# JanLohse/raw2film

Measured on AMD Instinct MI355X. Metric: megapixels/sec full film pipeline (neg+print+grain+halation+MTF), 100MP frame, higher is better.
Workload: dtype f32 (pointwise stages, grain) + f64 (FFT stencils; the MTF's scratch images are complex64)

## Files before the change

### raw2film_amd/csrc/r2f_fft.hip

```cpp
#include <algorithm>

#include "r2f_launch.h"
#include "r2f_fft_math.h"

#include "../../include/r2f.h"

namespace r2f {

constexpr int kN = kFftN;
constexpr int kFftThreads = 256;
constexpr int kTPitch = 17;
constexpr int kTLine = 16 * kTPitch;

#ifndef R2F_FFT_EXPT
#define R2F_FFT_EXPT 0
#endif
template <bool INV>
__device__ __forceinline__ void fft256(cplx (&v)[16], const cplx w1, double* tbuf, int lane) {
    dft16<INV>(v);
    twiddle_powers<INV>(v, w1);
    if (R2F_FFT_EXPT & 1) {
        dft16<INV>(v);
        return;
    }
// ... 119 lines not shown
    __builtin_amdgcn_wave_barrier();
#pragma unroll
    for (int i = 0; i < 16; ++i) v[i] = make_double2(re[i], rd[4 * i]);
    __builtin_amdgcn_wave_barrier();
    dft16<INV>(v);
    const cplx wh = make_double2(h == 0 ? 1.0 : (h == 1 ? 0.9951847266721969 : (h == 2 ? 0.9807852804032304 : 0.9569403357322088)),
                                 h == 0 ? 0.0 : (h == 1 ? -0.0980171403295606 : (h == 2 ? -0.19509032201612825 : -0.2902846772544623)));
    twiddle_powers<INV>(v, wh);
    const bool upper = h & 2, odd = h & 1, rot = h == 3;
#pragma unroll
    for (int c = 0; c < 16; ++c) {
        cplx o = make_double2(swap_lane2(v[c].x), swap_lane2(v[c].y));
        cplx b = upper ? csub(o, v[c]) : cadd(v[c], o);
        if (rot) b = INV ? make_double2(-b.y, b.x) : make_double2(b.y, -b.x);
        o = make_double2(swap_lane1(b.x), swap_lane1(b.y));
        v[c] = odd ? csub(o, b) : cadd(b, o);
    }
}

__device__ __forceinline__ bool window_of(const FftConvArgs& a, int t, int& wy, int& wx) {
    if (t >= a.ntiles) return false;
    const int ty = a.y0 + (t / a.gx) * a.vy, tx = (t % a.gx) * a.vx;
    wy = ty - a.ay;
    wx = tx - a.ax;
    return true;
}

__device__ __forceinline__ double* wave_tbuf(double* smem) { return smem + (threadIdx.x >> 6) * 4 * kTLine; }

__device__ __forceinline__ unsigned sidx(int r, int k, int nbx) {
    return (unsigned)((((r >> 4) * nbx + (k >> 4)) << 8) + ((((k >> 2) & 3) * 16 + (r & 15)) << 2) + (k & 3));
}

__device__ __forceinline__ cplx& at(cplx* base, unsigned idx) {
    return *reinterpret_cast<cplx*>(reinterpret_cast<char*>(base) + (idx << 4));
}
__device__ __forceinline__ const cplx& at(const cplx* base, unsigned idx) {
    return *reinterpret_cast<const cplx*>(reinterpret_cast<const char*>(base) + (idx << 4));
}

struct __attribute__((packed, aligned(4))) C96 {
    unsigned hr, hi;
    unsigned lo;
};
template <int ST>
__device__ __forceinline__ cplx sld(const void* base, unsigned idx) {
    if (ST == 1) {
        const float2 v = *reinterpret_cast<const float2*>(reinterpret_cast<const char*>(base) + (idx << 3));
        return make_double2((double)v.x, (double)v.y);
    }
    if (ST == 2) {
        const C96 e = *reinterpret_cast<const C96*>(reinterpret_cast<const char*>(base) + idx * 12u);
        return make_double2(__hiloint2double((int)e.hr, (int)(e.lo << 16)), __hiloint2double((int)e.hi, (int)(e.lo & 0xffff0000u)));
    }
    return *reinterpret_cast<const cplx*>(reinterpret_cast<const char*>(base) + (idx << 4));
}
template <int ST>
__device__ __forceinline__ void sst(void* base, unsigned idx, const cplx v) {
    if (ST == 1)
        *reinterpret_cast<float2*>(reinterpret_cast<char*>(base) + (idx << 3)) = make_float2((float)v.x, (float)v.y);
    else if (ST == 2) {
        const unsigned long long br = (unsigned long long)__double_as_longlong(v.x) + 0x8000ull;
        const unsigned long long bi = (unsigned long long)__double_as_longlong(v.y) + 0x8000ull;
        C96 e;
        e.hr = (unsigned)(br >> 32), e.hi = (unsigned)(bi >> 32);
        e.lo = ((unsigned)br >> 16) | ((unsigned)bi & 0xffff0000u);
        *reinterpret_cast<C96*>(reinterpret_cast<char*>(base) + idx * 12u) = e;
    } else
        *reinterpret_cast<cplx*>(reinterpret_cast<char*>(base) + (idx << 4)) = v;
}
__device__ __forceinline__ bool pair_packed(const FftConvArgs& a, int pc) { return a.dyn_flags[pc] != 0; }

template <int ST>
__device__ __forceinline__ char* simg(double2* s1, long long pair, long long n) {
    return reinterpret_cast<char*>(s1) + pair * n * (ST == 1 ? 8 : (ST == 2 ? 12 : 16));
}

#ifndef R2F_DECIDE_OWN_COLUMNS_ONLY
#define R2F_DECIDE_OWN_COLUMNS_ONLY 0
#endif
__device__ __forceinline__ void reflected_reach(int w0, int n, int size, int& lo, int& hi) {
    const int last = size - 1, w1 = w0 + n - 1;
    lo = max(w0, 0), hi = min(w1, last);
    if (w0 < 0) hi = max(hi, min(-w0, last));
    if (w1 > last) lo = min(lo, max(2 * last - w1, 0));
}
__global__ __launch_bounds__(256) void fft_decide_kernel(const FftConvArgs a, const RangeRecord rec, const float bound, const float floor_, int* flags) {
    const int pc = blockIdx.x * 256 + threadIdx.x;
    if (pc >= a.ppc) return;
    int lo = (int)kFrameMinReset, hi = 0;
    bool known = rec.tiles != nullptr && !(rec.blk && rec.blk->e_max == 0x7f800000u);
    for (int half = 0; half < 2 && known; ++half) {
        int wy, wx;
        if (!window_of(a, 2 * pc + half, wy, wx)) continue;
        const int b0 = a.src.gy0, b1 = a.src.gy0 + a.src.rows - 1;
        const int r0 = clampi(max(wy, 0), b0, b1), r1 = clampi(min(wy + a.ny - 1, a.H_global - 1), b0, b1);
        int c0, c1;
        reflected_reach(wx, a.nx, a.W, c0, c1);
#if R2F_DECIDE_OWN_COLUMNS_ONLY
        c0 = max(wx, 0), c1 = min(wx + a.nx - 1, a.W - 1);
#endif
        for (int ty = r0 >> kRangeTileRowsLog2; ty <= (r1 >> kRangeTileRowsLog2); ++ty)
// ... 4 lines not shown
                }
                const int2 t = rec.tiles[(long long)ty * rec.txn + tx];
                if (t.x == (int)kFrameMinReset && t.y == (int)kFrameMaxReset) known = false;
                lo = min(lo, t.x), hi = max(hi, t.y);
            }
    }
    const float flo = __int_as_float(lo), fhi = __int_as_float(hi);
    flags[pc] = (known && fhi <= bound * fmaxf(flo, floor_)) ? 1 : 0;
}

#ifndef R2F_FFT_EXP
#define R2F_FFT_EXP 0
#endif
template <int XL>
struct RowGeom {
    static constexpr int NX = 256 << XL, NBX = NX / 16, LPL = 16 << XL, ROWS = kFftThreads / LPL;
    static __device__ __forceinline__ int out_col(int l, int q) {
        return XL == 2 ? (l >> 2) + 16 * q + 256 * (((l & 1) << 1) | ((l >> 1) & 1)) : (XL == 1 ? 256 * (l & 1) + 16 * q + (l >> 1) : l + 16 * q);
    }
    static __device__ __forceinline__ double* line_buf(double* wave_buf, int lane) {
        return XL == 2 ? wave_buf : wave_buf + (XL == 1 ? (lane >> 5) * kTLine512 : (lane >> 4) * kTLine);
    }
    template <bool INV>
    static __device__ __forceinline__ void fft(cplx (&v)[16], const FftConvArgs& a, int l, double* wave_buf, int lane) {
        if (XL == 2)
            fft1024<INV>(v, a.tw1024[l], wave_buf, lane);
        else if (XL == 1)
            fft512<INV>(v, a.tw512[l], wave_buf, lane);
        else
            fft256<INV>(v, a.tw[l], wave_buf, lane);
    }
};

template <int XL, int ST>
__device__ __forceinline__ void fft_rows_fwd_body(const FftConvArgs& a, double* fsm) {
    typedef RowGeom<XL> G;
    constexpr int NX = G::NX, LPL = G::LPL;
    const int lane = threadIdx.x & 63, l = lane & (LPL - 1);
    unsigned tid0 = threadIdx.x;
    asm volatile("" : "+v"(tid0));
    const int pair = blockIdx.y, r = blockIdx.x * G::ROWS + tid0 / LPL;
    int wyA = 0, wxA = 0, wyB = 0, wxB = 0;
    const int gp = a.pair0 + pair, ci = gp / a.ppc, pc = gp - ci * a.ppc;
    const bool hasA = window_of(a, 2 * pc, wyA, wxA), hasB = window_of(a, 2 * pc + 1, wyB, wxB);
    const float* src = a.src.data + (long long)a.chan[ci] * a.src.plane_stride;
    if (R2F_FFT_EXP & 8) {
        const int above = pair - (a.gx + 1) / 2;
        if ((int)(blockIdx.x + 1) * G::ROWS <= a.ny - a.vy && above >= 0 && (a.pair0 + above) / a.ppc == ci && !a.raw) return;
    }
    cplx v[16];
    if (R2F_FFT_EXP & 1) {
#pragma unroll
        for (int m = 0; m < 16; ++m) v[m] = make_double2(1.0 + m + l, 0.5 * r);
    } else if (a.raw) {
#pragma unroll
        for (int m = 0; m < 16; ++m) v[m] = make_double2((double)src[(long long)r * NX + l + LPL * m], 0.0);
    } else {
        const float* rowA = src;
        const float* rowB = src;
        if (hasA) {
            const int sy = reflect101(wyA + r, a.H_global) - a.src.gy0;
            rowA = src + (long long)clampi(sy, 0, a.src.rows - 1) * a.W;
        }
        if (hasB) {
            const int sy = reflect101(wyB + r, a.H_global) - a.src.gy0;
            rowB = src + (long long)clampi(sy, 0, a.src.rows - 1) * a.W;
        }
        const bool inA = wxA >= 0 && wxA + NX <= a.W, inB = wxB >= 0 && wxB + NX <= a.W;
        float fa[16], fb[16];
#pragma unroll
        for (int m = 0; m < 16; ++m) fa[m] = fb[m] = 0.f;
        if (hasA) {
            if (inA) {
                const float* pa = rowA + wxA + l;
#pragma unroll
                for (int m = 0; m < 16; ++m) fa[m] = pa[LPL * m];
            } else {
#pragma unroll
                for (int m = 0; m < 16; ++m) fa[m] = rowA[reflect101(wxA + l + LPL * m, a.W)];
            }
        }
        if (hasB) {
            if (inB) {
                const float* pb = rowB + wxB + l;
#pragma unroll
                for (int m = 0; m < 16; ++m) fb[m] = pb[LPL * m];
            } else {
#pragma unroll
                for (int m = 0; m < 16; ++m) fb[m] = rowB[reflect101(wxB + l + LPL * m, a.W)];
            }
        }
#pragma unroll
        for (int m = 0; m < 16; ++m) v[m] = make_double2(__builtin_isfinite(fa[m]) ? (double)fa[m] : 0.0, __builtin_isfinite(fb[m]) ? (double)fb[m] : 0.0);
    }
    bool packed = false;
    if (ST == 3) packed = pair_packed(a, pc);
    if (!(R2F_FFT_EXP & 4)) {
        G::template fft<false>(v, a, l, wave_tbuf(fsm), lane);
    }
    unsigned tid = threadIdx.x;
    asm volatile("" : "+v"(tid));
    const int rs = blockIdx.x * G::ROWS + tid / LPL;
    const unsigned sb = sidx(rs, G::out_col(l, 0), G::NBX);
    if (ST == 3) {
        char* s1 = simg<3>(a.s1, pair, (long long)a.ny * NX);
        if (packed) {
#pragma unroll
            for (int q = 0; q < 16; ++q) sst<2>(s1, sb + q * 256, v[q]);
        } else {
#pragma unroll
            for (int q = 0; q < 16; ++q) sst<0>(s1, sb + q * 256, v[q]);
        }
        return;
    }
    constexpr int STS = ST == 3 ? 0 : ST;
    char* s1 = simg<STS>(a.s1, pair, (long long)a.ny * NX);
    if (R2F_FFT_EXP & 2) {
        if (v[3].x == 1.2345e300) sst<STS>(s1, 0, v[5]);
        return;
    }
#pragma unroll
    for (int q = 0; q < 16; ++q) sst<STS>(s1, sb + q * 256, v[q]);
    if (R2F_FFT_EXP & 8) {
        const int below = pair + (a.gx + 1) / 2;
        if (r >= a.vy && below < a.npairs && (a.pair0 + below) / a.ppc == ci && !a.raw) {
            char* s2 = simg<STS>(a.s1, below, (long long)a.ny * NX);
#pragma unroll
            for (int q = 0; q < 16; ++q) sst<STS>(s2, sidx(r - a.vy, G::out_col(l, q), G::NBX), v[q]);
        }
    }
}

#ifndef R2F_FFT_WPE1
#define R2F_FFT_WPE1 4
#endif
template <int XL, int ST>
__global__ __launch_bounds__(kFftThreads) __attribute__((amdgpu_waves_per_eu(R2F_FFT_WPE1, 8))) void fft_rows_fwd_kernel(const FftConvArgs a) {
    extern __shared__ __attribute__((aligned(16))) double fsm[];
    fft_rows_fwd_body<XL, ST>(a, fsm);
}

#ifndef R2F_FFT_EXP2
#define R2F_FFT_EXP2 0
#endif
__device__ __forceinline__ double& rat(cplx* base, unsigned idx) {
    return *reinterpret_cast<double*>(reinterpret_cast<char*>(base) + (idx << 3));
}
__device__ __forceinline__ double rat(const cplx* base, unsigned idx) {
    return *reinterpret_cast<const double*>(reinterpret_cast<const char*>(base) + (idx << 3));
}

template <int NBX, int ST, bool KR>
__device__ __forceinline__ void fft_cols_body(const FftConvArgs& a, const int mode, double* fsm) {
    const int lane = threadIdx.x & 63, l = lane & 15;
    const int pair = blockIdx.y, k = blockIdx.x * 16 + (threadIdx.x >> 4);
    char* s1 = simg<ST>(a.s1, pair, (long long)kN * (NBX * 16));
    const cplx* kf = a.kfs[(a.pair0 + pair) / a.ppc];
#ifndef R2F_FFT_KR_EARLY
#define R2F_FFT_KR_EARLY 0
#endif
    constexpr bool kEarly = (R2F_FFT_KR_EARLY >> (ST == 1 ? 1 : 0)) & 1;
    double kr[16];
    if (KR && kEarly && mode != 1) {
#pragma unroll
        for (int q = 0; q < 16; ++q) kr[q] = (R2F_FFT_EXP2 & 4) ? 0.5 + 0.25 * q : rat(kf, sidx(l + 16 * q, k, NBX));
    }
    cplx v[16];
#pragma unroll
    for (int m = 0; m < 16; ++m) v[m] = (R2F_FFT_EXP2 & 1) ? make_double2(1.0 + m + l, 0.5 * k) : sld<ST>(s1, sidx(l + 16 * m, k, NBX));
    const cplx w1 = a.tw[l];
    double* tbuf = wave_tbuf(fsm);
    fft256<false>(v, w1, tbuf, lane);
    if (mode == 1) {
        const double sc = R2F_FFT_EPI2 ? 1.0 / ((double)kN * (NBX * 16)) : 1.0;
#pragma unroll
        for (int q = 0; q < 16; ++q) {
            if (KR)
                rat(a.kf_out, sidx(l + 16 * q, k, NBX)) = v[q].x * sc;
            else
                at(a.kf_out, sidx(l + 16 * q, k, NBX)) = make_double2(v[q].x * sc, -v[q].y * sc);
        }
        return;
    }
    if (KR) {
        if (!kEarly) {
#pragma unroll
            for (int q = 0; q < 16; ++q) kr[q] = (R2F_FFT_EXP2 & 4) ? 0.5 + 0.25 * q : rat(kf, sidx(l + 16 * q, k, NBX));
        }
#pragma unroll
        for (int q = 0; q < 16; ++q) v[q] = make_double2(v[q].x * kr[q], v[q].y * kr[q]);
    } else {
#pragma unroll
        for (int q = 0; q < 16; ++q) v[q] = cmul(v[q], (R2F_FFT_EXP2 & 4) ? make_double2(0.5, 0.25 * q) : at(kf, sidx(l + 16 * q, k, NBX)));
    }
    fft256<true>(v, w1, tbuf, lane);
    if (R2F_FFT_EXP2 & 2) {
        if (v[3].x == 1.2345e300) sst<ST>(s1, 0, v[5]);
        return;
    }
#pragma unroll
    for (int q = 0; q < 16; ++q)
        if ((unsigned)(l + 16 * q - a.oy) < (unsigned)a.vy) sst<ST>(s1, sidx(l + 16 * q, k, NBX), v[q]);
}

template <int NBX, int ST, bool KR>
__device__ __forceinline__ void fft_cols_y512_body(const FftConvArgs& a, const int mode, double* fsm) {
    const int lane = threadIdx.x & 63, l = lane & 31;
    const int pair = blockIdx.y, k = blockIdx.x * 8 + (threadIdx.x >> 5);
    char* s1 = simg<ST>(a.s1, pair, (long long)512 * (NBX * 16));
    cplx v[16];
#pragma unroll
    for (int m = 0; m < 16; ++m) v[m] = sld<ST>(s1, sidx(l + 32 * m, k, NBX));
    const cplx w1 = a.tw512[l];
    double* tbuf = wave_tbuf(fsm);
    fft512<false>(v, w1, tbuf, lane);
    const cplx* kf = a.kfs[(a.pair0 + pair) / a.ppc];
    const int f0 = 256 * (l & 1) + (l >> 1);
    if (mode == 1) {
        const double sc = R2F_FFT_EPI2 ? 1.0 / (512.0 * (NBX * 16)) : 1.0;
#pragma unroll
        for (int q = 0; q < 16; ++q) {
            if (KR)
                rat(a.kf_out, sidx(f0 + 16 * q, k, NBX)) = v[q].x * sc;
            else
                at(a.kf_out, sidx(f0 + 16 * q, k, NBX)) = make_double2(v[q].x * sc, -v[q].y * sc);
        }
        return;
    }
    if (KR) {
        double kr[16];
#pragma unroll
        for (int q = 0; q < 16; ++q) kr[q] = rat(kf, sidx(f0 + 16 * q, k, NBX));
#pragma unroll
        for (int q = 0; q < 16; ++q) v[q] = make_double2(v[q].x * kr[q], v[q].y * kr[q]);
    } else {
#pragma unroll
        for (int q = 0; q < 16; ++q) v[q] = cmul(v[q], at(kf, sidx(f0 + 16 * q, k, NBX)));
    }
    fft512_rev<true>(v, w1, tbuf, lane);
#pragma unroll
    for (int q = 0; q < 16; ++q)
        if ((unsigned)(l + 32 * q - a.oy) < (unsigned)a.vy) sst<ST>(s1, sidx(l + 32 * q, k, NBX), v[q]);
}

#ifndef R2F_FFT_WPE2
#define R2F_FFT_WPE2 2
#endif
template <int NBX, bool Y512, int ST, bool KR>
__global__ __launch_bounds__(kFftThreads) __attribute__((amdgpu_waves_per_eu(R2F_FFT_WPE2, 8))) void fft_cols_kernel(const FftConvArgs a, const int mode) {
    extern __shared__ __attribute__((aligned(16))) double fsm[];
    if (Y512)
        fft_cols_y512_body<NBX, ST, KR>(a, mode, fsm);
    else
        fft_cols_body<NBX, ST, KR>(a, mode, fsm);
}


template <int NBX, int ST>
__device__ __forceinline__ void fft_cols_walk_body(const FftConvArgs& a, double* fsm) {
    const int lane = threadIdx.x & 63, l = lane & 15;
    const int k = blockIdx.x * 16 + (threadIdx.x >> 4);
    double* tbuf = wave_tbuf(fsm);
    const long long img = (long long)kN * (NBX * 16);
    const int G = gridDim.y;
    const cplx w1 = a.tw[l];
    double kr[16];
    int ci_have = -1;
    for (int pair = blockIdx.y; pair < a.npairs; pair += G) {
        const int gp = a.pair0 + pair, ci = gp / a.ppc;
        const bool packed = ST == 3 ? pair_packed(a, gp - ci * a.ppc) : false;
        char* s1 = simg<ST>(a.s1, pair, img);
        unsigned sbase = sidx(l, k, NBX);
        cplx w = w1;
        asm volatile("" : "+v"(w.x), "+v"(w.y), "+v"(sbase));
        if (ci != ci_have) {
// ... 16 lines not shown
#pragma unroll
            for (int m = 0; m < 16; ++m) v[m] = sld<STL>(s1, sbase + m * (NBX * 256));
        }
        fft256<false>(v, w, tbuf, lane);
#pragma unroll
        for (int q = 0; q < 16; ++q) v[q] = make_double2(v[q].x * kr[q], v[q].y * kr[q]);
        asm volatile("" : "+v"(w.x), "+v"(w.y));
        fft256<true>(v, w, tbuf, lane);
        if (ST == 3) {
            if (packed) {
#pragma unroll
                for (int q = 0; q < 16; ++q)
                    if ((unsigned)(l + 16 * q - a.oy) < (unsigned)a.vy) sst<2>(s1, sbase + q * (NBX * 256), v[q]);
            } else {
#pragma unroll
                for (int q = 0; q < 16; ++q)
                    if ((unsigned)(l + 16 * q - a.oy) < (unsigned)a.vy) sst<0>(s1, sbase + q * (NBX * 256), v[q]);
            }
        } else {
            constexpr int STS = ST == 3 ? 0 : ST;
#pragma unroll
            for (int q = 0; q < 16; ++q)
                if ((unsigned)(l + 16 * q - a.oy) < (unsigned)a.vy) sst<STS>(s1, sbase + q * (NBX * 256), v[q]);
        }
    }
}

template <int NBX, int ST>
__global__ __launch_bounds__(kFftThreads) __attribute__((amdgpu_waves_per_eu(2, 2))) void fft_cols_walk_kernel(const FftConvArgs a) {
    extern __shared__ __attribute__((aligned(16))) double fsm[];
    fft_cols_walk_body<NBX, ST>(a, fsm);
}

#ifndef R2F_FFT_EXP3
#define R2F_FFT_EXP3 0
#endif
#ifndef R2F_FFT_CURVE_BATCH
#define R2F_FFT_CURVE_BATCH 4
#endif
template <int XL, int EPI, int ST>
__device__ __forceinline__ void fft_rows_inv_body(const FftConvArgs& a, double* fsm) {
    typedef RowGeom<XL> G;
    constexpr int NX = G::NX, LPL = G::LPL;
    const int lane = threadIdx.x & 63, l = lane & (LPL - 1);
    const int pair = blockIdx.y, r = (a.oy & ~(G::ROWS - 1)) + blockIdx.x * G::ROWS + threadIdx.x / LPL, ro = r - a.oy;
    const bool live = (unsigned)ro < (unsigned)a.vy;
    bool packed = false;
    if (ST == 3) packed = pair_packed(a, (a.pair0 + pair) % a.ppc);
    float4* cells_lds = reinterpret_cast<float4*>(fsm + a.epi_lds_off);
    if (EPI == 2) {
        const int gp0 = a.pair0 + pair, ch0 = a.chan[gp0 / a.ppc];
        const float4* src_cells = a.curve.cells + (long long)ch0 * (a.curve.m - 1);
        for (int i = threadIdx.x; i < a.curve.m - 1; i += kFftThreads) cells_lds[i] = src_cells[i];
        __syncthreads();
    }
    cplx v[16];
    if (R2F_FFT_EXP3 & 1) {
#pragma unroll
        for (int m = 0; m < 16; ++m) v[m] = make_double2(1.0 + m + l, 0.5 * r);
    } else if (ST == 3) {
        const char* s1 = simg<3>(a.s1, pair, (long long)a.ny * NX);
        if (packed) {
#pragma unroll
            for (int m = 0; m < 16; ++m) v[m] = sld<2>(s1, sidx(live ? r : a.oy, l + LPL * m, G::NBX));
        } else {
#pragma unroll
            for (int m = 0; m < 16; ++m) v[m] = sld<0>(s1, sidx(live ? r : a.oy, l + LPL * m, G::NBX));
        }
    } else {
        constexpr int STL = ST == 3 ? 0 : ST;
        const char* s1 = simg<STL>(a.s1, pair, (long long)a.ny * NX);
#pragma unroll
        for (int m = 0; m < 16; ++m) v[m] = sld<STL>(s1, sidx(live ? r : a.oy, l + LPL * m, G::NBX));
    }
    if (!(R2F_FFT_EXP3 & 4)) {
        G::template fft<true>(v, a, l, wave_tbuf(fsm), lane);
    }
    if (!live) return;
    if (R2F_FFT_EXP3 & 2) {
        if (v[3].x == 1.2345e300) a.dst.data[0] = (float)v[5].y;
        return;
    }
    const int gp = a.pair0 + pair, ci = gp / a.ppc, pc = gp - ci * a.ppc, ch = a.chan[ci];
    float* dplane = a.dst.data + (long long)ch * a.dst.plane_stride;
    const double scale = R2F_FFT_EPI2 ? 1.0 : 1.0 / ((double)NX * a.ny);
#pragma unroll
    for (int half = 0; half < 2; ++half) {
        int wy, wx;
        if (!window_of(a, 2 * pc + half, wy, wx)) continue;
        const int gy = wy + a.ay + ro;
        if (gy >= a.y1) continue;
        float* dbase = dplane + (long long)(gy - a.dst.gy0) * a.W + wx + a.ax;
        float o[16];
#pragma unroll
        for (int q = 0; q < 16; ++q) o[q] = R2F_FFT_EPI2 ? (float)(half ? v[q].y : v[q].x) : (float)((half ? v[q].y : v[q].x) * scale);
        if (EPI) {
            constexpr int CB = R2F_FFT_CURVE_BATCH;
#pragma unroll
            for (int b = 0; b < 16 / CB; ++b) {
                float ob[CB];
#ifndef R2F_FFT_EPI_ABLATE
#define R2F_FFT_EPI_ABLATE 0
#endif
#pragma unroll
                for (int q = 0; q < CB; ++q) ob[q] = (R2F_FFT_EPI_ABLATE & 6) ? o[CB * b + q] * 0.5f : log10_fast(o[CB * b + q], a.log_eps);
                if (R2F_FFT_EPI_ABLATE & 5) {
// ... 4 lines not shown
#pragma unroll
                for (int q = 0; q < CB; ++q) o[CB * b + q] = ob[q];
            }
        }
        const int c_end = min(a.vx, a.W - (wx + a.ax));
        if (a.vec4) {
            float* tf = reinterpret_cast<float*>(G::line_buf(wave_tbuf(fsm), lane)) + ((a.ox + 3) & ~3);
#pragma unroll
            for (int q = 0; q < 16; ++q) tf[G::out_col(l, q) - a.ox] = o[q];
            __builtin_amdgcn_wave_barrier();
#pragma unroll
            for (int j = 0; j < 4; ++j) {
                const int c = 4 * (l + LPL * j);
                const float4 val = *reinterpret_cast<const float4*>(tf + c);
                if (c < c_end) st4_stream(dbase + c, val);
            }
            __builtin_amdgcn_wave_barrier();
        } else {
#pragma unroll
            for (int q = 0; q < 16; ++q)
                if ((unsigned)(G::out_col(l, q) - a.ox) < (unsigned)c_end) dbase[G::out_col(l, q) - a.ox] = o[q];
        }
    }
}

#ifndef R2F_FFT_WPE3
#define R2F_FFT_WPE3 3
#endif
template <int XL, int EPI, int ST>
__global__ __launch_bounds__(kFftThreads) __attribute__((amdgpu_waves_per_eu(EPI ? R2F_FFT_WPE3 : (XL ? 3 : 4), 8))) void fft_rows_inv_kernel(const FftConvArgs a) {
    extern __shared__ __attribute__((aligned(16))) double fsm[];
    fft_rows_inv_body<XL, EPI, ST>(a, fsm);
}

static size_t fft_lds_bytes() { return (size_t)(kFftThreads / 64) * 4 * kTLine * sizeof(double); }


template <int XL>
static void launch_rows_fwd(const FftConvArgs& a, hipStream_t s) {
    const dim3 block(kFftThreads), grid(a.ny / RowGeom<XL>::ROWS, a.npairs);
    if (a.s32 == 1)
        launch_k((fft_rows_fwd_kernel<XL, 1>), grid, block, fft_lds_bytes(), s, a);
    else if (a.s32 == 3)
        launch_k((fft_rows_fwd_kernel<XL, 3>), grid, block, fft_lds_bytes(), s, a);
    else if (a.s32 == 2)
        launch_k((fft_rows_fwd_kernel<XL, 2>), grid, block, fft_lds_bytes(), s, a);
    else
        launch_k((fft_rows_fwd_kernel<XL, 0>), grid, block, fft_lds_bytes(), s, a);
}

hipError_t launch_fft_rows_fwd(const FftConvArgs& a, hipStream_t s) {
    if (a.nx == 1024)
        launch_rows_fwd<2>(a, s);
    else if (a.nx == 512)
        launch_rows_fwd<1>(a, s);
    else
        launch_rows_fwd<0>(a, s);
    return take_launch_status();
}

template <int NBX, bool Y512, bool KR>
static void launch_cols_kr(const FftConvArgs& a, int mode, hipStream_t s) {
    const dim3 block(kFftThreads), grid(a.nx / (Y512 ? 8 : 16), a.npairs);
    if (a.s32 == 1)
        launch_k((fft_cols_kernel<NBX, Y512, 1, KR>), grid, block, fft_lds_bytes(), s, a, mode);
    else if (a.s32 == 2)
        launch_k((fft_cols_kernel<NBX, Y512, 2, KR>), grid, block, fft_lds_bytes(), s, a, mode);
    else
        launch_k((fft_cols_kernel<NBX, Y512, 0, KR>), grid, block, fft_lds_bytes(), s, a, mode);
}

template <int NBX, bool Y512>
static void launch_cols(const FftConvArgs& a, int mode, hipStream_t s) {
    if (a.kreal)
        launch_cols_kr<NBX, Y512, true>(a, mode, s);
    else
        launch_cols_kr<NBX, Y512, false>(a, mode, s);
}

template <bool Y512>
static void launch_cols_nx(const FftConvArgs& a, int mode, hipStream_t s) {
    if (a.nx == 1024)
        launch_cols<64, Y512>(a, mode, s);
    else if (a.nx == 512)
        launch_cols<32, Y512>(a, mode, s);
    else
        launch_cols<16, Y512>(a, mode, s);
}

static bool cols_walk_applies(const FftConvArgs& a, int mode) { return a.cols_walk && mode == 0 && a.ny == 256 && a.kreal; }

template <int NBX>
static void launch_cols_walk_st(const FftConvArgs& a, dim3 grid, hipStream_t s) {
    const dim3 block(kFftThreads);
    if (a.s32 == 1)
        launch_k((fft_cols_walk_kernel<NBX, 1>), grid, block, fft_lds_bytes(), s, a);
    else if (a.s32 == 3)
        launch_k((fft_cols_walk_kernel<NBX, 3>), grid, block, fft_lds_bytes(), s, a);
    else if (a.s32 == 2)
        launch_k((fft_cols_walk_kernel<NBX, 2>), grid, block, fft_lds_bytes(), s, a);
    else
        launch_k((fft_cols_walk_kernel<NBX, 0>), grid, block, fft_lds_bytes(), s, a);
}

static void launch_cols_walk(const FftConvArgs& a, hipStream_t s) {
    const int cb = a.nx / 16, per = std::max(1, a.cols_slots / cb), iters = (a.npairs + per - 1) / per, G = (a.npairs + iters - 1) / iters;
    const dim3 grid(cb, G);
    if (a.nx == 1024)
        launch_cols_walk_st<64>(a, grid, s);
    else if (a.nx == 512)
        launch_cols_walk_st<32>(a, grid, s);
    else
        launch_cols_walk_st<16>(a, grid, s);
}

hipError_t fft_init_attributes() { return hipSuccess; }

hipError_t launch_fft_decide(const FftConvArgs& a, const RangeRecord& rec, float bound, float floor_, int* flags, hipStream_t s) {
    if (a.ppc <= 0) return hipSuccess;
    launch_k(fft_decide_kernel, dim3((a.ppc + 255) / 256), dim3(256), 0, s, a, rec, bound, floor_, flags);
    return take_launch_status();
}

hipError_t launch_fft_cols(const FftConvArgs& a, int mode, hipStream_t s) {
    if (cols_walk_applies(a, mode)) {
        launch_cols_walk(a, s);
        return take_launch_status();
    }
    if (a.ny == 512)
        launch_cols_nx<true>(a, mode, s);
    else
        launch_cols_nx<false>(a, mode, s);
    return take_launch_status();
}

template <int XL, int EPI>
static void launch_rows_inv(const FftConvArgs& a0, hipStream_t s) {
    const int rows = RowGeom<XL>::ROWS;
    const dim3 grid(((a0.oy & (rows - 1)) + a0.vy + rows - 1) / rows, a0.npairs);
    FftConvArgs a = a0;
    size_t lds = fft_lds_bytes();
    a.epi_lds_off = 0;
    if (EPI == 2) {
        a.epi_lds_off = (int)(lds / sizeof(double));
        lds += (size_t)(a.curve.m - 1) * sizeof(float4);
    }
    if (a.s32 == 1)
        launch_k((fft_rows_inv_kernel<XL, EPI, 1>), grid, dim3(kFftThreads), lds, s, a);
    else if (a.s32 == 3)
        launch_k((fft_rows_inv_kernel<XL, EPI, 3>), grid, dim3(kFftThreads), lds, s, a);
    else if (a.s32 == 2)
        launch_k((fft_rows_inv_kernel<XL, EPI, 2>), grid, dim3(kFftThreads), lds, s, a);
    else
        launch_k((fft_rows_inv_kernel<XL, EPI, 0>), grid, dim3(kFftThreads), lds, s, a);
}

template <int XL>
static void launch_rows_inv_epi(const FftConvArgs& a, hipStream_t s) {
    if (a.epilogue == 1 && a.epi_lds && a.curve.near && (size_t)(a.curve.m - 1) * sizeof(float4) + fft_lds_bytes() <= 53 * 1024)
        launch_rows_inv<XL, 2>(a, s);
    else if (a.epilogue == 1)
        launch_rows_inv<XL, 1>(a, s);
    else
        launch_rows_inv<XL, 0>(a, s);
}

hipError_t launch_fft_rows_inv(const FftConvArgs& a, hipStream_t s) {
    if (a.nx == 1024)
        launch_rows_inv_epi<2>(a, s);
    else if (a.nx == 512)
        launch_rows_inv_epi<1>(a, s);
    else
        launch_rows_inv_epi<0>(a, s);
    return take_launch_status();
}

}
```

### raw2film_amd/csrc/r2f_plan.cpp

```cpp
#include "r2f_plan.h"

#include "../../include/r2f.h"

#include <algorithm>
#include <cmath>
#include <cstdio>
#include <cstring>

namespace r2f {
namespace plan {

void tap_box(const Taps& t, int c, int box[4]) {
    int i_lo = t.kh, i_hi = -1, j_lo = t.kw, j_hi = -1;
    for (int i = 0; i < t.kh; ++i)
        for (int j = 0; j < t.kw; ++j)
            if (t.at(i, j, c) != 0.f) {
                i_lo = std::min(i_lo, i), i_hi = std::max(i_hi, i);
                j_lo = std::min(j_lo, j), j_hi = std::max(j_hi, j);
            }
    if (i_hi < 0) i_lo = i_hi = t.kh / 2, j_lo = j_hi = t.kw / 2;
    box[0] = i_lo, box[1] = i_hi, box[2] = j_lo, box[3] = j_hi;
}

bool single_tap_channel(const Taps& t, int c, float* w) {
// ... 175 lines not shown
    const int n = 2 * R + 1;
    for (int c = 0; c < 3; ++c) {
        int b[4];
        tap_box(t, c, b);
        if (b[1] - b[0] + 1 != n || b[3] - b[2] + 1 != n) return false;
        auto K = [&](int i, int j) { return (double)t.at(b[0] + i, b[2] + j, c); };
        const double centre = K(R, R);
        double kmax = 0.0;
        for (int i = 0; i < n; ++i)
            for (int j = 0; j < n; ++j) kmax = std::max(kmax, std::fabs(K(i, j)));
        if (!(centre > 0.0) || centre < 0.25 * kmax) return false;
        for (int i = 0; i < n; ++i) u[c][i] = (float)K(i, R);
        for (int j = 0; j <= R; ++j) v[c][j] = (float)(K(R, j) / centre);
        for (int i = 0; i < n; ++i)
            for (int j = 0; j < n; ++j) {
                const double vv = (double)v[c][j <= R ? j : 2 * R - j];
                if (std::fabs((double)u[c][i] * vv - K(i, j)) > 6e-7 * kmax) return false;
            }
    }
    return true;
}

void stencil_source_rows(int y0, int y1, int above, int below, int H, int* lo_out, int* hi_out) {
    int lo = y0 - above, hi = y1 - 1 + below;
    int need_lo = std::max(lo, 0), need_hi = std::min(hi, H - 1);
    if (H > 1) {
        if (lo < 0) need_hi = std::max(need_hi, std::min(-lo, H - 1));
        if (hi > H - 1) need_lo = std::min(need_lo, std::max(2 * (H - 1) - hi, 0));
    }
    *lo_out = need_lo;
    *hi_out = need_hi + 1;
}

bool fft_window(const FftOptions& o, int bh, int bw, int W, int H, bool s32, int* ny, int* nx) {
    double best = -1.0;
    const int window_max = bw > 200 ? std::max(o.window_max, 512) : o.window_max;
    for (int y = 256; y <= 512; y *= 2) {
        if (bh > 200 ? y != 512 : (o.window_rows && y != o.window_rows)) continue;
        for (int x = 256; x <= 1024; x *= 2) {
            if (x > window_max && x != o.window) continue;
            if (bw > 200 ? (x < 512 || (o.window >= 512 && x != o.window)) : (o.window && x != o.window)) continue;
            const int vy = y - bh + 1, vx = (x - bw + 1) & ~3;
            if (vy < 1 || vx < 4) continue;
            const double n = (double)y * x, part = n * vy / y;
            const double p2 = y == 512 ? 1.3 : 1.0;
            const double e = s32 ? 4.0 : 8.0;
            const double bytes = 4.0 * n + e * n + p2 * (e * n + e * part) + e * part + 4.0 * vy * vx;
            const double cost = (double)((W + vx - 1) / vx) * ((H + vy - 1) / vy) * bytes;
            if (best < 0.0 || cost < best) best = cost, *ny = y, *nx = x;
        }
    }
    return best >= 0.0;
}

FftBatches fft_batches(const FftOptions& o, int ny, int nx, int bh, int bw, int W, int y0, int y1, int nch, int elem_bytes) {
    FftBatches b;
    b.ny = ny, b.nx = nx;
    b.vy = ny - bh + 1;
    b.vx = (nx - bw + 1) & ~3;
    if (b.vy < 1 || b.vx < 4 || nch < 1 || y1 <= y0 || W < 1) return b;
    b.gx = (W + b.vx - 1) / b.vx;
    b.ntiles = b.gx * ((y1 - y0 + b.vy - 1) / b.vy);
    b.ppc = (b.ntiles + 1) / 2;
    b.pairs = b.ppc * nch;
    b.img_bytes = (size_t)ny * nx * (size_t)elem_bytes;
    const int fft_batch = std::max(1, (int)(((size_t)std::max(o.batch_mib, 1) << 20) / b.img_bytes));
    b.nstreams = b.pairs > fft_batch ? std::max(1, std::min(o.streams, 4)) : 1;
    b.batch = std::min(b.pairs, std::max(1, fft_batch / b.nstreams));
    if (o.even) {
        int nb = (b.pairs + b.batch - 1) / b.batch;
        nb = (nb + b.nstreams - 1) / b.nstreams * b.nstreams;
        b.batch = (b.pairs + nb - 1) / nb;
    }
    b.launches = (b.pairs + b.batch - 1) / b.batch;
    b.scratch_bytes = (size_t)b.batch * b.nstreams * b.img_bytes;
    return b;
}

std::vector<int> tile_order(int gx, int gy, int band) {
    const int nwg = gx * gy, q = nwg / 8, r = nwg % 8;
// ... 369 lines not shown
```

### raw2film_amd/csrc/r2f_stencil.hip

```cpp
#include <algorithm>
#include <cmath>
#include <cstring>

#include "r2f_ctx.h"

namespace r2f {

static_assert(plan::fixed_ax(4) == fixed_stencil_ax(4) && plan::fixed_ax(7) == fixed_stencil_ax(7) && plan::fixed_ax(11) == fixed_stencil_ax(11),
              "plan::fixed_ax restates fixed_stencil_ax");

int ensure_stencil(r2f_ctx* ctx, int which, int Q, int TW, int TH, size_t lds_budget, bool common_box) {
    const bool allow_sym = ctx->opt.sym != 0;
    StencilSet& s = ctx->stencil[which];
    if (!s.present) return fail(ctx, R2F_EINVAL, "stencil %d not set (r2f_set_kernel)", which);
    if (s.built_q == Q && s.built_tw == TW && s.built_th == TH && s.built_budget == lds_budget && s.common_box == common_box &&
        s.built_sym == allow_sym)
        return R2F_OK;
    const plan::Taps taps = s.taps();
    int box[3][4];
    for (int c = 0; c < 3; ++c) plan::tap_box(taps, c, box[c]);
    if (common_box) {
        for (int c = 1; c < 3; ++c) {
            box[0][0] = std::min(box[0][0], box[c][0]);
            box[0][1] = std::max(box[0][1], box[c][1]);
// ... 152 lines not shown
        if (ctx->fft.kf_valid[which][c][shape] && ctx->fft.kf_real[which][c][shape] == kreal) continue;
        const std::vector<float> kimg = plan::fft_kernel_image(set.taps(), c, b, ny, nx, kreal);
        rc = upload(ctx, ctx->fft.kimg, kimg.data(), img * sizeof(float));
        if (rc) return rc;
        rc = ctx->fft.kf[which][c][shape].reserve(ctx, img * sizeof(double2), Grow::SyncGeneration);
        if (rc) return rc;
        ctx->fft.kf_real[which][c][shape] = kreal;
        FftConvArgs k = a;
        k.src.data = static_cast<float*>(ctx->fft.kimg.p);
        k.raw = 1;
        k.s32 = 0;
        k.nch = 1, k.chan[0] = 0, k.ppc = 1;
        k.ntiles = 1, k.gx = 1, k.npairs = 1, k.pair0 = 0;
        k.s1 = static_cast<double2*>(ctx->fft.s1.p);
        k.kf_out = static_cast<double2*>(ctx->fft.kf[which][c][shape].p);
        R2F_HIP(ctx, launch_fft_rows_fwd(k, s));
        R2F_HIP(ctx, launch_fft_cols(k, 1, s));
        ctx->fft.kf_valid[which][c][shape] = true;
    }
    a.src = to_dev(src);
    a.dst = to_dev(dst);
    a.nch = nch;
    for (int i = 0; i < nch; ++i) {
        a.chan[i] = chans[i];
        a.kfs[i] = static_cast<const double2*>(ctx->fft.kf[which][chans[i]][shape].p);
    }
    a.y0 = y0, a.y1 = y1, a.W = W, a.H_global = H;
    a.s32 = ((ctx->opt.fft_s96 >> which) & 1) ? 2 : (s32_eff ? 1 : 0);
    for (int i = 0; i < nch; ++i)
        if (set.mixed_sign[chans[i]] && ctx->opt.fft_mixed_sign) a.s32 = 0;
    bool unit_gain = true;
    for (int i = 0; i < nch; ++i) unit_gain = unit_gain && set.unit_gain[chans[i]];
    if (a.s32 == 0 && which == R2F_KERNEL_HALATION && epilogue == 1 && dyn && ctx->opt.fft_s96_auto && a.kreal && unit_gain &&
        ny == 256 && ctx->opt.fft_cols_walk && ctx->curve.cells) {
        a.s32 = 3;
        ctx->frame_dyn_armed = true;
    }
    const plan::FftBatches fb = plan::fft_batches(fo, ny, nx, bh, bw, W, y0, y1, nch, a.s32 == 1 ? 8 : (a.s32 == 2 ? 12 : 16));
    a.gx = fb.gx;
    a.ntiles = fb.ntiles;
    a.ppc = fb.ppc;
    a.epilogue = epilogue;
    a.epi_lds = ctx->opt.fft_epi_lds;
    a.curve = ctx->curve;
    a.log_eps = log_eps;
    a.vec4 = planes_vec_ok(dst, W) ? 1 : 0;
    const size_t img_bytes = fb.img_bytes;
    const int pairs = fb.pairs, nstreams = fb.nstreams, batch = fb.batch;
    rc = ctx->fft.s1.reserve(ctx, fb.scratch_bytes, Grow::SyncGeneration);
    if (rc) return rc;
    if (a.s32 == 3) {
        rc = ensure_range_tiles(ctx, H, W);
        if (rc) return rc;
        rc = ctx->dyn_flags.reserve(ctx, (size_t)std::max(fb.ppc, 1) * sizeof(int), Grow::SyncGeneration);
        if (rc) return rc;
        float bound, floor_;
        dyn_rule(ctx, &bound, &floor_);
        a.dyn_flags = static_cast<const int*>(ctx->dyn_flags.p);
        ctx->dyn_flags_ppc = fb.ppc;
        R2F_HIP(ctx, launch_fft_decide(a, record_of(ctx), bound, floor_, static_cast<int*>(ctx->dyn_flags.p), s));
    }
    hipStream_t lanes[4] = {s, s, s, s};
    if (nstreams > 1) {
        for (int i = 0; i < nstreams; ++i) {
            if (!ctx->fft.stream[i]) R2F_HIP(ctx, hipStreamCreateWithFlags(&ctx->fft.stream[i], hipStreamNonBlocking));
            if (!ctx->fft.ev_out[i]) R2F_HIP(ctx, hipEventCreateWithFlags(&ctx->fft.ev_out[i], hipEventDisableTiming));
            lanes[i] = ctx->fft.stream[i];
// ... 157 lines not shown
```

Measured before the change: 21350.

## Add 512-row FFT scratch layout with paired column accesses and walk kernel

Introduces a dedicated scratch index layout for 512-row FFT windows that interleaves rows r and r+256 so column kernels can load and store two complex values per access. It adds 512-row variants of the row forward/inverse kernels and a persistent column-walk kernel, and enables dynamic packed 96-bit storage beyond 256-row windows. The window-cost model now applies a per-term penalty for 512-row windows, which can change which window shape the planner picks. This adds template instantiations and extra code paths, and the inverse rows kernel now launches over all 512 rows with early exits.

```diff
diff --git a/raw2film_amd/csrc/r2f_fft.hip b/raw2film_amd/csrc/r2f_fft.hip
--- a/raw2film_amd/csrc/r2f_fft.hip
+++ b/raw2film_amd/csrc/r2f_fft.hip
@@ -175,6 +175,18 @@
     return (unsigned)((((r >> 4) * nbx + (k >> 4)) << 8) + ((((k >> 2) & 3) * 16 + (r & 15)) << 2) + (k & 3));
 }
 
+__device__ __forceinline__ unsigned sidx512(int r, int k, int nbx) {
+    return (unsigned)((((((r >> 4) & 15) * nbx + (k >> 4)) << 9) + ((((k >> 1) & 7) * 16 + (r & 15)) << 2) + ((k & 1) << 1)) + (r >> 8));
+}
+template <bool Y512>
+__device__ __forceinline__ unsigned sidx_of(int r, int k, int nbx) {
+    return Y512 ? sidx512(r, k, nbx) : sidx(r, k, nbx);
+}
+template <bool Y512>
+__device__ __forceinline__ int rows_line(int wg, int li, int rows) {
+    return Y512 ? wg * (rows >> 1) + (li >> 1) + ((li & 1) << 8) : wg * rows + li;
+}
+
 __device__ __forceinline__ cplx& at(cplx* base, unsigned idx) {
     return *reinterpret_cast<cplx*>(reinterpret_cast<char*>(base) + (idx << 4));
 }
@@ -186,6 +198,9 @@
     unsigned hr, hi;
     unsigned lo;
 };
+__device__ __forceinline__ cplx unpack96(const C96 e) {
+    return make_double2(__hiloint2double((int)e.hr, (int)(e.lo << 16)), __hiloint2double((int)e.hi, (int)(e.lo & 0xffff0000u)));
+}
 template <int ST>
 __device__ __forceinline__ cplx sld(const void* base, unsigned idx) {
     if (ST == 1) {
@@ -193,24 +208,55 @@
         return make_double2((double)v.x, (double)v.y);
     }
     if (ST == 2) {
-        const C96 e = *reinterpret_cast<const C96*>(reinterpret_cast<const char*>(base) + idx * 12u);
-        return make_double2(__hiloint2double((int)e.hr, (int)(e.lo << 16)), __hiloint2double((int)e.hi, (int)(e.lo & 0xffff0000u)));
+        return unpack96(*reinterpret_cast<const C96*>(reinterpret_cast<const char*>(base) + idx * 12u));
     }
     return *reinterpret_cast<const cplx*>(reinterpret_cast<const char*>(base) + (idx << 4));
+}
+__device__ __forceinline__ C96 pack96(const cplx v) {
+    const unsigned long long br = (unsigned long long)__double_as_longlong(v.x) + 0x8000ull;
+    const unsigned long long bi = (unsigned long long)__double_as_longlong(v.y) + 0x8000ull;
+    C96 e;
+    e.hr = (unsigned)(br >> 32), e.hi = (unsigned)(bi >> 32);
+    e.lo = ((unsigned)br >> 16) | ((unsigned)bi & 0xffff0000u);
+    return e;
 }
 template <int ST>
 __device__ __forceinline__ void sst(void* base, unsigned idx, const cplx v) {
     if (ST == 1)
         *reinterpret_cast<float2*>(reinterpret_cast<char*>(base) + (idx << 3)) = make_float2((float)v.x, (float)v.y);
+    else if (ST == 2)
+        *reinterpret_cast<C96*>(reinterpret_cast<char*>(base) + idx * 12u) = pack96(v);
+    else
+        *reinterpret_cast<cplx*>(reinterpret_cast<char*>(base) + (idx << 4)) = v;
+}
+struct __attribute__((packed, aligned(8))) C96x2 {
+    C96 a, b;
+};
+template <int ST>
+__device__ __forceinline__ void sld2(const void* base, unsigned idx, cplx& a, cplx& b) {
+    if (ST == 1) {
+        const float4 v = *reinterpret_cast<const float4*>(reinterpret_cast<const char*>(base) + (idx << 3));
+        a = make_double2((double)v.x, (double)v.y), b = make_double2((double)v.z, (double)v.w);
+    } else if (ST == 2) {
+        const C96x2 e = *reinterpret_cast<const C96x2*>(reinterpret_cast<const char*>(base) + idx * 12u);
+        a = unpack96(e.a), b = unpack96(e.b);
+    } else {
+        const cplx* p = reinterpret_cast<const cplx*>(reinterpret_cast<const char*>(base) + (idx << 4));
+        a = p[0], b = p[1];
+    }
+}
+template <int ST>
+__device__ __forceinline__ void sst2(void* base, unsigned idx, const cplx a, const cplx b) {
+    if (ST == 1)
+        *reinterpret_cast<float4*>(reinterpret_cast<char*>(base) + (idx << 3)) = make_float4((float)a.x, (float)a.y, (float)b.x, (float)b.y);
     else if (ST == 2) {
-        const unsigned long long br = (unsigned long long)__double_as_longlong(v.x) + 0x8000ull;
-        const unsigned long long bi = (unsigned long long)__double_as_longlong(v.y) + 0x8000ull;
-        C96 e;
-        e.hr = (unsigned)(br >> 32), e.hi = (unsigned)(bi >> 32);
-        e.lo = ((unsigned)br >> 16) | ((unsigned)bi & 0xffff0000u);
-        *reinterpret_cast<C96*>(reinterpret_cast<char*>(base) + idx * 12u) = e;
-    } else
-        *reinterpret_cast<cplx*>(reinterpret_cast<char*>(base) + (idx << 4)) = v;
+        C96x2 e;
+        e.a = pack96(a), e.b = pack96(b);
+        *reinterpret_cast<C96x2*>(reinterpret_cast<char*>(base) + idx * 12u) = e;
+    } else {
+        cplx* p = reinterpret_cast<cplx*>(reinterpret_cast<char*>(base) + (idx << 4));
+        p[0] = a, p[1] = b;
+    }
 }
 __device__ __forceinline__ bool pair_packed(const FftConvArgs& a, int pc) { return a.dyn_flags[pc] != 0; }
 
@@ -281,14 +327,15 @@
     }
 };
 
-template <int XL, int ST>
+template <int XL, int ST, bool Y512 = false>
 __device__ __forceinline__ void fft_rows_fwd_body(const FftConvArgs& a, double* fsm) {
     typedef RowGeom<XL> G;
     constexpr int NX = G::NX, LPL = G::LPL;
+    constexpr unsigned kBlk = Y512 ? 512 : 256;
     const int lane = threadIdx.x & 63, l = lane & (LPL - 1);
     unsigned tid0 = threadIdx.x;
     asm volatile("" : "+v"(tid0));
-    const int pair = blockIdx.y, r = blockIdx.x * G::ROWS + tid0 / LPL;
+    const int pair = blockIdx.y, r = rows_line<Y512>(blockIdx.x, tid0 / LPL, G::ROWS);
     int wyA = 0, wxA = 0, wyB = 0, wxB = 0;
     const int gp = a.pair0 + pair, ci = gp / a.ppc, pc = gp - ci * a.ppc;
     const bool hasA = window_of(a, 2 * pc, wyA, wxA), hasB = window_of(a, 2 * pc + 1, wyB, wxB);
@@ -349,16 +396,16 @@
     }
     unsigned tid = threadIdx.x;
     asm volatile("" : "+v"(tid));
-    const int rs = blockIdx.x * G::ROWS + tid / LPL;
-    const unsigned sb = sidx(rs, G::out_col(l, 0), G::NBX);
+    const int rs = rows_line<Y512>(blockIdx.x, tid / LPL, G::ROWS);
+    const unsigned sb = sidx_of<Y512>(rs, G::out_col(l, 0), G::NBX);
     if (ST == 3) {
         char* s1 = simg<3>(a.s1, pair, (long long)a.ny * NX);
         if (packed) {
 #pragma unroll
-            for (int q = 0; q < 16; ++q) sst<2>(s1, sb + q * 256, v[q]);
+            for (int q = 0; q < 16; ++q) sst<2>(s1, sb + q * kBlk, v[q]);
         } else {
 #pragma unroll
-            for (int q = 0; q < 16; ++q) sst<0>(s1, sb + q * 256, v[q]);
+            for (int q = 0; q < 16; ++q) sst<0>(s1, sb + q * kBlk, v[q]);
         }
         return;
     }
@@ -369,13 +416,13 @@
         return;
     }
 #pragma unroll
-    for (int q = 0; q < 16; ++q) sst<STS>(s1, sb + q * 256, v[q]);
+    for (int q = 0; q < 16; ++q) sst<STS>(s1, sb + q * kBlk, v[q]);
     if (R2F_FFT_EXP & 8) {
         const int below = pair + (a.gx + 1) / 2;
         if (r >= a.vy && below < a.npairs && (a.pair0 + below) / a.ppc == ci && !a.raw) {
             char* s2 = simg<STS>(a.s1, below, (long long)a.ny * NX);
 #pragma unroll
-            for (int q = 0; q < 16; ++q) sst<STS>(s2, sidx(r - a.vy, G::out_col(l, q), G::NBX), v[q]);
+            for (int q = 0; q < 16; ++q) sst<STS>(s2, sidx_of<Y512>(r - a.vy, G::out_col(l, q), G::NBX), v[q]);
         }
     }
 }
@@ -387,6 +434,11 @@
 __global__ __launch_bounds__(kFftThreads) __attribute__((amdgpu_waves_per_eu(R2F_FFT_WPE1, 8))) void fft_rows_fwd_kernel(const FftConvArgs a) {
     extern __shared__ __attribute__((aligned(16))) double fsm[];
     fft_rows_fwd_body<XL, ST>(a, fsm);
+}
+template <int XL, int ST>
+__global__ __launch_bounds__(kFftThreads) __attribute__((amdgpu_waves_per_eu(R2F_FFT_WPE1, 8))) void fft_rows_fwd512_kernel(const FftConvArgs a) {
+    extern __shared__ __attribute__((aligned(16))) double fsm[];
+    fft_rows_fwd_body<XL, ST, true>(a, fsm);
 }
 
 #ifndef R2F_FFT_EXP2
@@ -452,44 +504,64 @@
         if ((unsigned)(l + 16 * q - a.oy) < (unsigned)a.vy) sst<ST>(s1, sidx(l + 16 * q, k, NBX), v[q]);
 }
 
+constexpr unsigned cols512_step(int nbx) { return (unsigned)nbx * 1024u; }
+
+template <int ST, int NBX>
+__device__ __forceinline__ void cols512_load(const char* s1, unsigned sbase, cplx (&v)[16]) {
+#pragma unroll
+    for (int m = 0; m < 8; ++m) sld2<ST>(s1, sbase + m * cols512_step(NBX), v[m], v[m + 8]);
+}
+template <int ST, int NBX>
+__device__ __forceinline__ void cols512_store(const FftConvArgs& a, char* s1, unsigned sbase, int l, const cplx (&v)[16]) {
+#pragma unroll
+    for (int q = 0; q < 8; ++q) {
+        const bool lo = (unsigned)(l + 32 * q - a.oy) < (unsigned)a.vy, hi = (unsigned)(l + 32 * q + 256 - a.oy) < (unsigned)a.vy;
+        const unsigned i = sbase + q * cols512_step(NBX);
+        if (lo && hi)
+            sst2<ST>(s1, i, v[q], v[q + 8]);
+        else if (lo)
+            sst<ST>(s1, i, v[q]);
+        else if (hi)
+            sst<ST>(s1, i + 1, v[q + 8]);
+    }
+}
+
 template <int NBX, int ST, bool KR>
 __device__ __forceinline__ void fft_cols_y512_body(const FftConvArgs& a, const int mode, double* fsm) {
     const int lane = threadIdx.x & 63, l = lane & 31;
     const int pair = blockIdx.y, k = blockIdx.x * 8 + (threadIdx.x >> 5);
     char* s1 = simg<ST>(a.s1, pair, (long long)512 * (NBX * 16));
+    const unsigned sbase = sidx512(l, k, NBX);
     cplx v[16];
-#pragma unroll
-    for (int m = 0; m < 16; ++m) v[m] = sld<ST>(s1, sidx(l + 32 * m, k, NBX));
+    cols512_load<ST, NBX>(s1, sbase, v);
     const cplx w1 = a.tw512[l];
     double* tbuf = wave_tbuf(fsm);
     fft512<false>(v, w1, tbuf, lane);
     const cplx* kf = a.kfs[(a.pair0 + pair) / a.ppc];
-    const int f0 = 256 * (l & 1) + (l >> 1);
+    const unsigned fbase = sidx512(256 * (l & 1) + (l >> 1), k, NBX);
     if (mode == 1) {
         const double sc = R2F_FFT_EPI2 ? 1.0 / (512.0 * (NBX * 16)) : 1.0;
 #pragma unroll
         for (int q = 0; q < 16; ++q) {
             if (KR)
-                rat(a.kf_out, sidx(f0 + 16 * q, k, NBX)) = v[q].x * sc;
+                rat(a.kf_out, fbase + q * (NBX * 512)) = v[q].x * sc;
             else
-                at(a.kf_out, sidx(f0 + 16 * q, k, NBX)) = make_double2(v[q].x * sc, -v[q].y * sc);
+                at(a.kf_out, fbase + q * (NBX * 512)) = make_double2(v[q].x * sc, -v[q].y * sc);
         }
         return;
     }
     if (KR) {
         double kr[16];
 #pragma unroll
-        for (int q = 0; q < 16; ++q) kr[q] = rat(kf, sidx(f0 + 16 * q, k, NBX));
+        for (int q = 0; q < 16; ++q) kr[q] = rat(kf, fbase + q * (NBX * 512));
 #pragma unroll
         for (int q = 0; q < 16; ++q) v[q] = make_double2(v[q].x * kr[q], v[q].y * kr[q]);
     } else {
 #pragma unroll
-        for (int q = 0; q < 16; ++q) v[q] = cmul(v[q], at(kf, sidx(f0 + 16 * q, k, NBX)));
+        for (int q = 0; q < 16; ++q) v[q] = cmul(v[q], at(kf, fbase + q * (NBX * 512)));
     }
     fft512_rev<true>(v, w1, tbuf, lane);
-#pragma unroll
-    for (int q = 0; q < 16; ++q)
-        if ((unsigned)(l + 32 * q - a.oy) < (unsigned)a.vy) sst<ST>(s1, sidx(l + 32 * q, k, NBX), v[q]);
+    cols512_store<ST, NBX>(a, s1, sbase, l, v);
 }
 
 #ifndef R2F_FFT_WPE2
@@ -572,18 +644,79 @@
     fft_cols_walk_body<NBX, ST>(a, fsm);
 }
 
+template <int NBX, int ST>
+__device__ __forceinline__ void fft_cols_walk512_body(const FftConvArgs& a, double* fsm) {
+    const int lane = threadIdx.x & 63, l = lane & 31;
+    const int k = blockIdx.x * 8 + (threadIdx.x >> 5);
+    double* tbuf = wave_tbuf(fsm);
+    const long long img = (long long)512 * (NBX * 16);
+    const int G = gridDim.y;
+    const cplx w1 = a.tw512[l];
+    double kr[16];
+    int ci_have = -1;
+    for (int pair = blockIdx.y; pair < a.npairs; pair += G) {
+        const int gp = a.pair0 + pair, ci = gp / a.ppc;
+        const bool packed = ST == 3 ? pair_packed(a, gp - ci * a.ppc) : false;
+        char* s1 = simg<ST>(a.s1, pair, img);
+        unsigned sbase = sidx512(l, k, NBX);
+        cplx w = w1;
+        asm volatile("" : "+v"(w.x), "+v"(w.y), "+v"(sbase));
+        if (ci != ci_have) {
+            const cplx* kf = a.kfs[ci];
+            const unsigned fbase = sidx512(256 * (l & 1) + (l >> 1), k, NBX);
+#pragma unroll
+            for (int q = 0; q < 16; ++q) kr[q] = rat(kf, fbase + q * (NBX * 512));
+            ci_have = ci;
+        }
+        cplx v[16];
+        if (ST == 3) {
+            if (packed)
+                cols512_load<2, NBX>(s1, sbase, v);
+            else
+                cols512_load<0, NBX>(s1, sbase, v);
+        } else {
+            cols512_load<(ST == 3 ? 0 : ST), NBX>(s1, sbase, v);
+        }
+        fft512<false>(v, w, tbuf, lane);
+#pragma unroll
+        for (int q = 0; q < 16; ++q) v[q] = make_double2(v[q].x * kr[q], v[q].y * kr[q]);
+        asm volatile("" : "+v"(w.x), "+v"(w.y));
+        fft512_rev<true>(v, w, tbuf, lane);
+        if (ST == 3) {
+            if (packed)
+                cols512_store<2, NBX>(a, s1, sbase, l, v);
+            else
+                cols512_store<0, NBX>(a, s1, sbase, l, v);
+        } else {
+            cols512_store<(ST == 3 ? 0 : ST), NBX>(a, s1, sbase, l, v);
+        }
+    }
+}
+
+template <int NBX, int ST>
+__global__ __launch_bounds__(kFftThreads) __attribute__((amdgpu_waves_per_eu(2, 2))) void fft_cols_walk512_kernel(const FftConvArgs a) {
+    extern __shared__ __attribute__((aligned(16))) double fsm[];
+    fft_cols_walk512_body<NBX, ST>(a, fsm);
+}
+
 #ifndef R2F_FFT_EXP3
 #define R2F_FFT_EXP3 0
 #endif
 #ifndef R2F_FFT_CURVE_BATCH
 #define R2F_FFT_CURVE_BATCH 4
 #endif
-template <int XL, int EPI, int ST>
+template <int XL, int EPI, int ST, bool Y512 = false>
 __device__ __forceinline__ void fft_rows_inv_body(const FftConvArgs& a, double* fsm) {
     typedef RowGeom<XL> G;
     constexpr int NX = G::NX, LPL = G::LPL;
     const int lane = threadIdx.x & 63, l = lane & (LPL - 1);
-    const int pair = blockIdx.y, r = (a.oy & ~(G::ROWS - 1)) + blockIdx.x * G::ROWS + threadIdx.x / LPL, ro = r - a.oy;
+    if (Y512) {
+        const int lo = blockIdx.x * (G::ROWS / 2), end = a.oy + a.vy;
+        if (!(lo < end && lo + G::ROWS / 2 > a.oy) && !(lo + 256 < end && lo + 256 + G::ROWS / 2 > a.oy)) return;
+    }
+    const int pair = blockIdx.y;
+    const int r = Y512 ? rows_line<true>(blockIdx.x, threadIdx.x / LPL, G::ROWS) : (a.oy & ~(G::ROWS - 1)) + blockIdx.x * G::ROWS + threadIdx.x / LPL;
+    const int ro = r - a.oy;
     const bool live = (unsigned)ro < (unsigned)a.vy;
     bool packed = false;
     if (ST == 3) packed = pair_packed(a, (a.pair0 + pair) % a.ppc);
@@ -602,16 +735,16 @@
         const char* s1 = simg<3>(a.s1, pair, (long long)a.ny * NX);
         if (packed) {
 #pragma unroll
-            for (int m = 0; m < 16; ++m) v[m] = sld<2>(s1, sidx(live ? r : a.oy, l + LPL * m, G::NBX));
+            for (int m = 0; m < 16; ++m) v[m] = sld<2>(s1, sidx_of<Y512>(live ? r : a.oy, l + LPL * m, G::NBX));
         } else {
 #pragma unroll
-            for (int m = 0; m < 16; ++m) v[m] = sld<0>(s1, sidx(live ? r : a.oy, l + LPL * m, G::NBX));
+            for (int m = 0; m < 16; ++m) v[m] = sld<0>(s1, sidx_of<Y512>(live ? r : a.oy, l + LPL * m, G::NBX));
         }
     } else {
         constexpr int STL = ST == 3 ? 0 : ST;
         const char* s1 = simg<STL>(a.s1, pair, (long long)a.ny * NX);
 #pragma unroll
-        for (int m = 0; m < 16; ++m) v[m] = sld<STL>(s1, sidx(live ? r : a.oy, l + LPL * m, G::NBX));
+        for (int m = 0; m < 16; ++m) v[m] = sld<STL>(s1, sidx_of<Y512>(live ? r : a.oy, l + LPL * m, G::NBX));
     }
     if (!(R2F_FFT_EXP3 & 4)) {
         G::template fft<true>(v, a, l, wave_tbuf(fsm), lane);
@@ -682,6 +815,11 @@
     extern __shared__ __attribute__((aligned(16))) double fsm[];
     fft_rows_inv_body<XL, EPI, ST>(a, fsm);
 }
+template <int XL, int EPI, int ST>
+__global__ __launch_bounds__(kFftThreads) __attribute__((amdgpu_waves_per_eu(EPI ? R2F_FFT_WPE3 : (XL ? 3 : 4), 8))) void fft_rows_inv512_kernel(const FftConvArgs a) {
+    extern __shared__ __attribute__((aligned(16))) double fsm[];
+    fft_rows_inv_body<XL, EPI, ST, true>(a, fsm);
+}
 
 static size_t fft_lds_bytes() { return (size_t)(kFftThreads / 64) * 4 * kTLine * sizeof(double); }
 
@@ -689,6 +827,17 @@
 template <int XL>
 static void launch_rows_fwd(const FftConvArgs& a, hipStream_t s) {
     const dim3 block(kFftThreads), grid(a.ny / RowGeom<XL>::ROWS, a.npairs);
+    if (a.ny == 512) {
+        if (a.s32 == 1)
+            launch_k((fft_rows_fwd512_kernel<XL, 1>), grid, block, fft_lds_bytes(), s, a);
+        else if (a.s32 == 3)
+            launch_k((fft_rows_fwd512_kernel<XL, 3>), grid, block, fft_lds_bytes(), s, a);
+        else if (a.s32 == 2)
+            launch_k((fft_rows_fwd512_kernel<XL, 2>), grid, block, fft_lds_bytes(), s, a);
+        else
+            launch_k((fft_rows_fwd512_kernel<XL, 0>), grid, block, fft_lds_bytes(), s, a);
+        return;
+    }
     if (a.s32 == 1)
         launch_k((fft_rows_fwd_kernel<XL, 1>), grid, block, fft_lds_bytes(), s, a);
     else if (a.s32 == 3)
@@ -738,11 +887,22 @@
         launch_cols<16, Y512>(a, mode, s);
 }
 
-static bool cols_walk_applies(const FftConvArgs& a, int mode) { return a.cols_walk && mode == 0 && a.ny == 256 && a.kreal; }
+static bool cols_walk_applies(const FftConvArgs& a, int mode) { return a.cols_walk && mode == 0 && (a.ny == 256 || a.ny == 512) && a.kreal; }
 
 template <int NBX>
 static void launch_cols_walk_st(const FftConvArgs& a, dim3 grid, hipStream_t s) {
     const dim3 block(kFftThreads);
+    if (a.ny == 512) {
+        if (a.s32 == 1)
+            launch_k((fft_cols_walk512_kernel<NBX, 1>), grid, block, fft_lds_bytes(), s, a);
+        else if (a.s32 == 3)
+            launch_k((fft_cols_walk512_kernel<NBX, 3>), grid, block, fft_lds_bytes(), s, a);
+        else if (a.s32 == 2)
+            launch_k((fft_cols_walk512_kernel<NBX, 2>), grid, block, fft_lds_bytes(), s, a);
+        else
+            launch_k((fft_cols_walk512_kernel<NBX, 0>), grid, block, fft_lds_bytes(), s, a);
+        return;
+    }
     if (a.s32 == 1)
         launch_k((fft_cols_walk_kernel<NBX, 1>), grid, block, fft_lds_bytes(), s, a);
     else if (a.s32 == 3)
@@ -754,7 +914,7 @@
 }
 
 static void launch_cols_walk(const FftConvArgs& a, hipStream_t s) {
-    const int cb = a.nx / 16, per = std::max(1, a.cols_slots / cb), iters = (a.npairs + per - 1) / per, G = (a.npairs + iters - 1) / iters;
+    const int cb = a.nx / (a.ny == 512 ? 8 : 16), per = std::max(1, a.cols_slots / cb), iters = (a.npairs + per - 1) / per, G = (a.npairs + iters - 1) / iters;
     const dim3 grid(cb, G);
     if (a.nx == 1024)
         launch_cols_walk_st<64>(a, grid, s);
@@ -787,7 +947,7 @@
 template <int XL, int EPI>
 static void launch_rows_inv(const FftConvArgs& a0, hipStream_t s) {
     const int rows = RowGeom<XL>::ROWS;
-    const dim3 grid(((a0.oy & (rows - 1)) + a0.vy + rows - 1) / rows, a0.npairs);
+    const dim3 grid(a0.ny == 512 ? 512 / rows : ((a0.oy & (rows - 1)) + a0.vy + rows - 1) / rows, a0.npairs);
     FftConvArgs a = a0;
     size_t lds = fft_lds_bytes();
     a.epi_lds_off = 0;
@@ -795,6 +955,17 @@
         a.epi_lds_off = (int)(lds / sizeof(double));
         lds += (size_t)(a.curve.m - 1) * sizeof(float4);
     }
+    if (a.ny == 512) {
+        if (a.s32 == 1)
+            launch_k((fft_rows_inv512_kernel<XL, EPI, 1>), grid, dim3(kFftThreads), lds, s, a);
+        else if (a.s32 == 3)
+            launch_k((fft_rows_inv512_kernel<XL, EPI, 3>), grid, dim3(kFftThreads), lds, s, a);
+        else if (a.s32 == 2)
+            launch_k((fft_rows_inv512_kernel<XL, EPI, 2>), grid, dim3(kFftThreads), lds, s, a);
+        else
+            launch_k((fft_rows_inv512_kernel<XL, EPI, 0>), grid, dim3(kFftThreads), lds, s, a);
+        return;
+    }
     if (a.s32 == 1)
         launch_k((fft_rows_inv_kernel<XL, EPI, 1>), grid, dim3(kFftThreads), lds, s, a);
     else if (a.s32 == 3)
diff --git a/raw2film_amd/csrc/r2f_plan.cpp b/raw2film_amd/csrc/r2f_plan.cpp
--- a/raw2film_amd/csrc/r2f_plan.cpp
+++ b/raw2film_amd/csrc/r2f_plan.cpp
@@ -231,6 +231,10 @@
     *hi_out = need_hi + 1;
 }
 
+#ifndef R2F_FFT_ROWS512_PRICED
+#define R2F_FFT_ROWS512_PRICED 1
+#endif
+constexpr double kP1Rows512 = R2F_FFT_ROWS512_PRICED ? 1.19 : 1.0, kP2Rows512 = R2F_FFT_ROWS512_PRICED ? 1.19 : 1.0, kP3Rows512 = R2F_FFT_ROWS512_PRICED ? 1.2 : 1.0;
 bool fft_window(const FftOptions& o, int bh, int bw, int W, int H, bool s32, int* ny, int* nx) {
     double best = -1.0;
     const int window_max = bw > 200 ? std::max(o.window_max, 512) : o.window_max;
@@ -242,9 +246,9 @@
             const int vy = y - bh + 1, vx = (x - bw + 1) & ~3;
             if (vy < 1 || vx < 4) continue;
             const double n = (double)y * x, part = n * vy / y;
-            const double p2 = y == 512 ? 1.3 : 1.0;
+            const double p1 = y == 512 ? kP1Rows512 : 1.0, p2 = y == 512 ? kP2Rows512 : 1.0, p3 = y == 512 ? kP3Rows512 : 1.0;
             const double e = s32 ? 4.0 : 8.0;
-            const double bytes = 4.0 * n + e * n + p2 * (e * n + e * part) + e * part + 4.0 * vy * vx;
+            const double bytes = p1 * (4.0 * n + e * n) + p2 * (e * n + e * part) + p3 * (e * part + 4.0 * vy * vx);
             const double cost = (double)((W + vx - 1) / vx) * ((H + vy - 1) / vy) * bytes;
             if (best < 0.0 || cost < best) best = cost, *ny = y, *nx = x;
         }
diff --git a/raw2film_amd/csrc/r2f_stencil.hip b/raw2film_amd/csrc/r2f_stencil.hip
--- a/raw2film_amd/csrc/r2f_stencil.hip
+++ b/raw2film_amd/csrc/r2f_stencil.hip
@@ -208,7 +208,7 @@
     bool unit_gain = true;
     for (int i = 0; i < nch; ++i) unit_gain = unit_gain && set.unit_gain[chans[i]];
     if (a.s32 == 0 && which == R2F_KERNEL_HALATION && epilogue == 1 && dyn && ctx->opt.fft_s96_auto && a.kreal && unit_gain &&
-        ny == 256 && ctx->opt.fft_cols_walk && ctx->curve.cells) {
+        ctx->opt.fft_cols_walk && ctx->curve.cells) {
         a.s32 = 3;
         ctx->frame_dyn_armed = true;
     }
```

Result: no change. 21380, median of 4 (+0.2%).
